# Naxaes/Rust-Swift-Raytracer

Hardware: AMD Instinct MI355X
Metric: Mrays/sec + frames/sec at 1920×1080 spp=64; 1/2/4/8 MI355X (higher is better)
Workload: dtype f32; 1 GPU; c2: 1920x1080, spp 64, depth 8, 486 spheres, 0 triangles, COUNTER RNG; width=1920, height=1080, spp=64, depth=8, parallelism=one device renders the frame in place (no RCCL call)

## Files before the change

include/raytracer_amd.h:

```cpp
#ifndef RAYTRACER_AMD_H
#define RAYTRACER_AMD_H

#include "raytracer.h"

#ifdef __cplusplus
extern "C" {
#endif

enum { RT_RNG_COUNTER = 1, RT_RNG_REPLAY = 2, RT_RNG_SERIAL = 3 };

typedef struct RtRenderOptions {
  int32_t samples_per_pixel;
  int32_t max_ray_bounces;
  uint32_t rng_mode;
  uint32_t seed;
  const uint32_t *replay_states;
  uint32_t row_block;
  uint32_t rank;
  uint32_t nranks;
  int32_t device;
  int32_t accel;
  uint32_t flags;
  int32_t ndevices;
} RtRenderOptions;
// ... 143 lines not shown
                         const void *d_records, float *d_out_rgb, void *d_out_rgba,
                         void *hip_stream);
int rt_filter_run(RtFilter *f, const RtFilterOptions *opts, const float *rgb,
                  const RtFirstHit *records, float *out_rgb, Rust_ColorU8 *out_pixels);
int rt_filter_accum(RtAccum *acc, const RtFilterOptions *opts, float *out_rgb,
                    Rust_ColorU8 *pixels);
int rt_filter_accum_device(RtAccum *acc, const RtFilterOptions *opts, float *d_out_rgb,
                           void *d_rgba, void *hip_stream);

long rt_read_samples(const Rust_WorldHandle *handle, int device, float *out, size_t n);

int rt_leaf_defer(const Rust_WorldHandle *handle, int device);

int rt_trace_plain(const Rust_WorldHandle *handle, int device);

int rt_trace_launched(const Rust_WorldHandle *handle, int device, unsigned char *out, size_t n,
                      int clear);
int rt_trace_instances(unsigned char *out, size_t n);

void rt_free_world(Rust_WorldHandle *handle);

const char *rt_last_error(void);

size_t rt_world_num_spheres(const Rust_WorldHandle *handle);
size_t rt_world_num_triangles(const Rust_WorldHandle *handle);
int rt_world_sphere(const Rust_WorldHandle *handle, size_t i, float out[10]);
int rt_world_triangle(const Rust_WorldHandle *handle, size_t i, float out[18]);
int rt_world_set_sphere_material(Rust_WorldHandle *handle, size_t i, const float material[6]);
int rt_world_set_triangle_material(Rust_WorldHandle *handle, size_t i, const float material[6]);
void rt_camera_get(const Rust_Camera *camera, float out[12]);
// ... 29 lines not shown
```

rust-swift-raytracer_amd/csrc/bvh.cpp:

```cpp
#include "bvh.h"

#include <algorithm>
#include <atomic>
#include <chrono>
#include <cmath>
#include <cstdio>
#include <cstdlib>
#include <cstring>
#include <limits>
#include <thread>

namespace rtamd {

namespace {

struct Box {
    double lo[3] = {std::numeric_limits<double>::infinity(), std::numeric_limits<double>::infinity(),
                    std::numeric_limits<double>::infinity()};
    double hi[3] = {-std::numeric_limits<double>::infinity(), -std::numeric_limits<double>::infinity(),
                    -std::numeric_limits<double>::infinity()};
    void grow(const Box &b) {
        for (int k = 0; k < 3; ++k) { lo[k] = std::min(lo[k], b.lo[k]); hi[k] = std::max(hi[k], b.hi[k]); }
    }
    void grow(const double p[3]) {
// ... 898 lines not shown
    double mag = 0;
    for (const Vec3 &v : cv) mag = std::max({mag, std::fabs((double)v.x), std::fabs((double)v.y),
                                             std::fabs((double)v.z)});
    double Mi[3][3];
    if (!(mag < 1e3) || !camera_inverse(cam, Mi)) return false;
    for (int r = 0; r < 3; ++r)
        for (int c = 0; c < 3; ++c) out.Mi[3 * r + c] = Mi[r][c];
    out.o[0] = cam.origin.x; out.o[1] = cam.origin.y; out.o[2] = cam.origin.z;
    out.e_abs = 4e-6 * (std::fabs(out.o[0]) + std::fabs(out.o[1]) + std::fabs(out.o[2]) + bv.mag);
    out.wden = (double)(float)(width - 1);
    out.hden = (double)(float)(height - 1);
    out.n = (uint32_t)n;
    out.width = (uint32_t)width;
    out.height = (uint32_t)height;
    return true;
}

PrimarySphereLists build_primary_sphere_lists(const SphereBVH &bv, const CameraModel &cam,
                                              size_t width, size_t height) {
    PrimarySphereLists out;
    const size_t n = bv.prims.size() / 4;
    if (n == 0 || n >= kSphListWalk || width < 2 || height < 2 || height > (1u << 24) ||
        width > (1u << 24) || width * height > (1ull << 28))
        return out;
    const Vec3 cv[4] = {cam.origin, cam.lower_left, cam.horizontal, cam.vertical};
    double mag = 0;
    for (const Vec3 &v : cv) mag = std::max({mag, std::fabs((double)v.x), std::fabs((double)v.y),
                                             std::fabs((double)v.z)});
    double Mi[3][3];
    if (!(mag < 1e3) || !camera_inverse(cam, Mi)) return out;
// ... 150 lines not shown
```

rust-swift-raytracer_amd/csrc/bvh.h:

```cpp
#pragma once

#include <cstdint>
#include <vector>

#include "scene.h"

namespace rtamd {

constexpr uint32_t kLeafBit = 0x80000000u;
constexpr uint32_t kNodeEnd = 0xFFFFFFFFu;

struct SphereBVH {
    std::vector<float> nodes;
    std::vector<uint32_t> miss;
    std::vector<float> prims;
    std::vector<uint32_t> prim_id;
    std::vector<uint32_t> big;
    float centre[3] = {0, 0, 0};
    float radius = 0, rmax = 0, mag = 0, inv_rmin = 0;
    uint32_t depth = 0;
    std::vector<uint32_t> corner;
};
constexpr uint32_t kCornerLeaf = 0x8000u, kCornerEnd = 0xFFFFu;
constexpr uint32_t kCornerMaxNodes = 0x7FFFu, kCornerMaxPrims = 0x1000u;
// ... 77 lines not shown
constexpr uint32_t kSphListWalk = 0xFFFFu;
struct PrimarySphereLists {
    std::vector<uint32_t> rec;
};
PrimarySphereLists build_primary_sphere_lists(const SphereBVH &bv, const CameraModel &cam,
                                              size_t width, size_t height);
struct SphereListParams {
    double Mi[9];
    double o[3];
    double e_abs, wden, hden;
    uint32_t n, width, height;
};
bool sphere_list_params(const SphereBVH &bv, const CameraModel &cam, size_t width, size_t height,
                        SphereListParams &out);

}
```

rust-swift-raytracer_amd/csrc/capi.cpp:

```cpp
#include <cstdio>
#include <cstdlib>
#include <cstring>
#include <string>

#include "../../include/raytracer.h"
#include "../../include/raytracer_amd.h"
#include "runtime.h"
#include "scene.h"

struct Rust_World {
    rtamd::WorldState state;
};
struct Rust_Camera {
    rtamd::CameraModel cam;
};
struct RtAccum {
    const Rust_WorldHandle *handle;
    rtamd::AccumState *state;
};
struct RtFilter {
    rtamd::FilterState *state;
};

namespace {
// ... 140 lines not shown
                                         static_cast<uint32_t *>(d_rgba),
                                         static_cast<hipStream_t>(hip_stream), stats);
    return rtamd::render_frame(h->world->state, h->camera->cam, width, height, o,
                               static_cast<uint32_t *>(d_rgba),
                               static_cast<hipStream_t>(hip_stream), stats);
}

int rt_trace_plain(const Rust_WorldHandle *h, int device) {
    if (!h || !h->world) {
        rtamd::set_error("rt_trace_plain: null argument");
        return -1;
    }
    return rtamd::trace_plain(h->world->state, device);
}

int rt_leaf_defer(const Rust_WorldHandle *h, int device) {
    if (!h || !h->world) {
        rtamd::set_error("rt_leaf_defer: null argument");
        return -1;
    }
    return rtamd::leaf_defer(h->world->state, device);
}

int rt_trace_launched(const Rust_WorldHandle *h, int device, unsigned char *out, size_t n, int clear) {
    if (!h || !h->world) {
        rtamd::set_error("rt_trace_launched: null argument");
        return -1;
    }
    return rtamd::trace_launched(h->world->state, device, out, n, clear != 0);
}
// ... 410 lines not shown
```

rust-swift-raytracer_amd/csrc/frame.cpp:

```cpp
#include <algorithm>
#include <cmath>
#include <cstdio>

#include "runtime_internal.h"

namespace rtamd {

size_t tile_rows(size_t height, uint32_t row_block, uint32_t rank, uint32_t nranks) {
    if (nranks <= 1) return height;
    const size_t B = row_block ? row_block : 1;
    const size_t blocks = (height + B - 1) / B;
    size_t rows = 0;
    for (size_t b = rank; b < blocks; b += nranks) rows += std::min(B, height - b * B);
    return rows;
}

size_t tile_row(size_t k, uint32_t row_block, uint32_t rank, uint32_t nranks) {
    if (nranks <= 1) return k;
    const size_t B = row_block ? row_block : 1;
    return ((k / B) * nranks + rank) * B + k % B;
}

void bind_scene_arrays(const DeviceState *d, const CameraModel &cam, size_t width, size_t height, TraceParams &p) {
    p.sph_hot = d->sph_hot.get(); p.sph_cold = d->sph_cold.get();
// ... 62 lines not shown
enum { kFrameRender = 0, kFrameNothing = 1, kFrameSerial = 2 };

struct LaunchPlan { uint64_t blocks, nwaves, chunk, parts, block_threads; };

struct FrameValues {
    uint32_t nranks = 1, B = 1;
    size_t T = 0;
    uint32_t spp = 0;
    uint64_t jobs_per_row = 0, slab_jobs = 0;
    size_t rows_per_slab = 0;
    bool fused = false, replay = false;
    bool use_bvh = false;
    const uint4 *corner_img = nullptr;
    TraceRequest want;
    bool primary_lists = false;
    bool use_tbvh = false;
    int ptl_where = 0;
    float inv_spp = 0.0f;
    bool timed = false;
    TraceVariant tv{};
    uint64_t waves_per_block = 0, full_blocks = 0, max_waves = 0;
};

struct LaunchesDone {
    LaunchPlan lean_plan{0, 0, 0, 0, 0};
    TraceVariant variant{};
    uint32_t launches = 0, waves = 0, nslab = 0;
    uint64_t samples = 0;
};

// ... 83 lines not shown
    if (f.use_bvh) {
        bind_sphere_tree(w, d, p);
        const bool lds_on = env_u64("RT_AMD_LDS", 1) != 0;
        if (lds_on && sp == nullptr && d->corner_bytes > 0 && env_u64("RT_AMD_CORNER", 1) != 0)
            f.corner_img = d->bvh_corner.get();
        f.want.corner = f.corner_img != nullptr;
        f.want.defer = f.want.corner && env_u64("RT_AMD_LEAF_DEFER", 1) != 0;
        f.want.plain = f.want.defer && d->plain_fits() && p.depth >= 1 && env_u64("RT_AMD_PLAIN", 1) != 0;
        p.use_lds = lds_on && (d->lds_bytes > 0 || f.corner_img != nullptr);
        if (d->ntri == 0 && env_u64("RT_AMD_SPHERE_LISTS", 1) != 0 && gpu_lists()) {
            bool ok = false;
            const int rc = device_sphere_lists(w, d, cam, width, height, s, ok);
            if (rc) return rc;
            p.spl = ok ? d->gspl.lists.get() : nullptr;
            f.primary_lists = ok;
        } else if (d->ntri == 0 && env_u64("RT_AMD_SPHERE_LISTS", 1) != 0 &&
                   prepare_primary_sphere_lists(w, cam, width, height)) {
            if (d->spl_version != w.spl_version) {
                HIP_TRY(replace_contents(d->spl, w.spl.rec));
                d->spl_version = w.spl_version;
            }
            p.spl = d->spl.get();
            f.primary_lists = p.spl != nullptr;
        }
    }
    return 0;
}

int bind_triangle_search(WorldState &w, DeviceState *d, const CameraModel &cam, size_t width, size_t height,
                         const RtRenderOptions &o, hipStream_t stream, hipStream_t s, FrameValues &f,
// ... 123 lines not shown
        if (const uint64_t bpc = env_u64("RT_AMD_BLOCKS_PER_CU", 0))
            if (tv.search != kSearchLdsCorner) blocks = (int)bpc;
        if (blocks < 1 && tv.lds()) { set_error("accumulation kernel does not fit its LDS tree"); return -1; }
        d->occupancy(tv) = std::max(blocks, 1);
    }
    f.waves_per_block = trace_block_threads(tv) / 64;
    f.full_blocks = (uint64_t)d->occupancy(tv) * (uint64_t)d->num_cus;
    f.max_waves = ap ? 0 : f.full_blocks * f.waves_per_block;
    p.stats = nullptr;
    if (f.timed && !ap) {
        HIP_TRY(d->stats.grow(f.max_waves * kStatSlots));
        HIP_TRY(hipMemsetAsync(d->stats.get(), 0, f.max_waves * kStatSlots * 8, s));
        p.stats = d->stats.get();
    }
    return 0;
}

hipError_t launch_recorded(DeviceState *d, TraceVariant v, const TraceParams &p, const TraceTail &tail,
                           uint32_t blocks, hipStream_t s) {
    const hipError_t e = launch_trace(v, p, tail, blocks, s);
    if (e == hipSuccess) d->trace_launched[trace_key(v)] = 1;
    return e;
}

int launch_serial_pass(DeviceState *d, size_t width, size_t height, const RtRenderOptions &o,
                       const SerialPass *sp, hipStream_t s, const FrameValues &f, TraceParams &p) {
    const uint32_t spp = f.spp;
    const uint64_t njobs = (uint64_t)sp->nsamples * sp->variants;
    if (njobs == 0) return 0;
    if (njobs > 0x7FFFFFFFull) { set_error("serial pass too large"); return -1; }
// ... 53 lines not shown

LaunchPlan plan_launch(DeviceState *d, const TraceParams &p, const FrameValues &f, TraceVariant v, uint64_t njobs) {
    const uint32_t spp = f.spp;
    const uint64_t wpb = trace_block_threads(v) / 64;
    const uint64_t jobs_per_block = wpb * 256;
    uint64_t blocks = std::min<uint64_t>((uint64_t)d->occupancy(v) * d->num_cus,
                                         (njobs + jobs_per_block - 1) / jobs_per_block);
    blocks = std::max<uint64_t>(blocks, 1);
    const uint64_t nwaves = blocks * wpb;
    uint64_t chunk = env_u64("RT_AMD_CHUNK", 0);
    if (!chunk) chunk = std::min<uint64_t>(256, std::max<uint64_t>(64, njobs / (nwaves * 16) / 64 * 64));
    chunk = chunk >= spp ? chunk / spp * spp : spp;
    if (f.fused) {
        uint64_t px = std::max<uint64_t>(1, std::min<uint64_t>(
            env_u64("RT_AMD_RESOLVE_PIX", p.step ? 1 : 8), 4096 / spp));
        while (px > 4 && njobs / (nwaves * px * spp) < 16) px /= 2;
        chunk = std::max<uint64_t>(chunk, px * spp);
    }
    uint64_t parts = env_u64("RT_AMD_PARTS", p.step ? 64 : 8);
    parts = std::max<uint64_t>(1, std::min<uint64_t>({parts, kMaxParts, njobs / (16 * chunk) + 1}));
    return LaunchPlan{blocks, nwaves, chunk, parts, wpb * 64};
}

int enqueue_launches(DeviceState *d, size_t width, size_t height, uint32_t *d_out, const AccumPass *ap,
                     hipStream_t s, const FrameValues &f, TraceParams &p, LaunchesDone &done) {
    const uint32_t spp = f.spp;
    const bool fused = f.fused, timed = f.timed, adapt = f.want.kind == kKindAdapt;
    TraceTail tail;
    tail.corner = f.corner_img;
    done.variant = f.tv;
    if (ap) {
// ... 2 lines not shown
        if (ap->n0 == 0) HIP_TRY(hipMemsetAsync(acc.sums.get(), 0, 3 * width * height * sizeof(float), s));
        tail.sums = acc.sums.get(), tail.n0 = ap->n0, tail.stride = acc.stride;
        if (adapt) tail.sumsq = acc.sumsq.get();
        if (adapt && ap->n0 == 0) {
            HIP_TRY(hipMemsetAsync(acc.sumsq.get(), 0, width * height * sizeof(float), s));
            HIP_TRY(hipMemsetAsync(acc.count.get(), 0, width * height * sizeof(uint32_t), s));
            HIP_TRY(launch_adapt_iota(const_cast<uint32_t *>(ap->list), (uint32_t)(width * height), s));
        }
    }
    const size_t units = adapt ? ap->nactive : f.T;
    const uint64_t jobs_per_unit = adapt ? spp : f.jobs_per_row;
    done.samples = (uint64_t)units * jobs_per_unit;
    const size_t units_per_slab =
        adapt ? (size_t)std::min<uint64_t>(std::max<uint64_t>(1, f.slab_jobs / spp), std::max<size_t>(units, 1))
              : f.rows_per_slab;
    uint32_t &nslab = done.nslab;
    for (size_t r0 = 0; r0 < units; r0 += units_per_slab, ++nslab) {
        const size_t rows = std::min(units_per_slab, units - r0);
        hipEvent_t *ev3 = nullptr;
        if (timed) {
            while (d->tev.size() < 3 * (size_t)(nslab + 1)) {
                hipEvent_t e;
                HIP_TRY(hipEventCreate(&e));
                d->tev.push_back(e);
            }
            ev3 = &d->tev[3 * (size_t)nslab];
        }
        const uint64_t njobs = rows * jobs_per_unit;
        p.slab_row0 = adapt ? 0u : (uint32_t)r0;
        p.gj32 = f.nranks == 1 && (uint64_t)width * height * spp < (1ull << 32) ? 1u : 0u;
        p.gj_c0 = (uint32_t)(((uint64_t)height - 1 - r0) * width * spp);
        p.gj_2p = (uint32_t)(2ull * width * spp);
        if (ap) p.gj32 = (uint64_t)width * height * ap->acc->stride < (1ull << 32) ? 1u : 0u;
// ... 124 lines not shown
    bind_scene(d, cam, width, height, o, sp, d_replay, f, p);
    rc = bind_sphere_search(w, d, cam, width, height, o, sp, s, f, p);
    if (rc) return rc;
    rc = bind_triangle_search(w, d, cam, width, height, o, stream, s, f, p);
    if (rc) return rc;
    const uint32_t nheld = ap ? ap->n0 + f.spp : f.spp;
    f.inv_spp = ap ? 1.0f / (float)nheld
                   : 1.0f / (float)o.samples_per_pixel;
    p.inv_spp = f.inv_spp;
    p.alpha_u8 = alpha_byte(nheld, f.inv_spp);
    p.out = d_out;
    f.timed = stats != nullptr;
    rc = choose_kernel_instance(d, sp, ap, s, f, p);
    if (rc) return rc;
    if (sp) return launch_serial_pass(d, width, height, o, sp, s, f, p);

    LaunchesDone done;
    rc = enqueue_launches(d, width, height, d_out, ap, s, f, p, done);
    if (rc) return rc;
    if (!f.timed) return 0;
    rc = queue_frame_stats(d, s, f, p, done);
    if (rc || defer_stats) return rc;
    return collect_frame_stats(d, stats);
}

int collect_frame_stats(DeviceState *d, RtRenderStats *stats) {
    auto &pd = d->pend;
    if (!pd.active) {
        set_error("no counted frame pending on this device");
        return -1;
    }
    pd.active = false;
    HIP_TRY(hipSetDevice(d->device));
    HIP_TRY(hipStreamSynchronize(pd.stream));
// ... 74 lines not shown
    std::lock_guard<std::recursive_mutex> lock(w.mu);
    DeviceState *d = nullptr;
    int rc = device_for(w, device, d);
    if (rc) return rc;
    return d->last_leaf_defer;
}

int trace_plain(WorldState &w, int device) {
    std::lock_guard<std::recursive_mutex> lock(w.mu);
    DeviceState *d = nullptr;
    int rc = device_for(w, device, d);
    if (rc) return rc;
    return d->last_plain ? 1 : 0;
}

int trace_launched(WorldState &w, int device, uint8_t *out, size_t n, bool clear) {
    std::lock_guard<std::recursive_mutex> lock(w.mu);
    DeviceState *d = nullptr;
    int rc = device_for(w, device, d);
    if (rc) return rc;
    if (out) std::memcpy(out, d->trace_launched, std::min<size_t>(n, kTraceKeys));
    if (clear) std::memset(d->trace_launched, 0, sizeof(d->trace_launched));
    return kTraceKeys;
}

int trace_instances(uint8_t *out, size_t n) {
    for (int key = 0; key < kTraceKeys && (size_t)key < n && out; ++key)
        out[key] = trace_instance_exists(key) ? 1 : 0;
    return kTraceKeys;
}
// ... 81 lines not shown
```

rust-swift-raytracer_amd/csrc/primary_lists.cpp:

```cpp
#include <chrono>

#include "runtime_internal.h"

namespace rtamd {

static uint32_t cam_leaf() {
    return (uint32_t)env_u64("RT_AMD_CAM_LEAF", 2);
}

void prepare_camera(WorldState &w, const CameraModel &cam, bool tree) {
    if (w.tbvh.nodes.empty() || env_u64("RT_AMD_CAMERA_TREE", 1) == 0) return;
    const float o[3] = {cam.origin.x, cam.origin.y, cam.origin.z};
    if (w.ctree_version && std::memcmp(o, w.ctree.origin, sizeof(o)) == 0 && (w.ctree_full || !tree)) return;
    w.ctree = build_camera_triangle_bvh(w.scene.triangles, w.packed.tri_hot, w.tbvh, o, cam_leaf(), tree);
    w.ctree_full = tree;
    ++w.ctree_version;
}

static bool sync_lists() { return env_u64("RT_AMD_SYNC_LISTS", 0) != 0; }
bool gpu_lists() { return env_u64("RT_AMD_GPU_LISTS", 1) != 0; }

template <typename T>
static bool job_ready(const std::future<T> &f) {
    return f.valid() && f.wait_for(std::chrono::seconds(0)) == std::future_status::ready;
// ... 58 lines not shown
                std::vector<uint32_t> dev(2 * width * height);
                HIP_TRY(hipMemcpyAsync(dev.data(), g.lists.get(), dev.size() * 4, hipMemcpyDeviceToHost, s));
                HIP_TRY(hipStreamSynchronize(s));
                for (size_t px = 0; px < width * height; ++px) {
                    const bool same = h.rec.empty()
                                          ? (dev[2 * px + 1] >> 16) == kSphListWalk
                                          : dev[2 * px] == h.rec[2 * px] && dev[2 * px + 1] == h.rec[2 * px + 1];
                    if (!same) {
                        set_error("RT_AMD_SPL_CHECK: device sphere lists differ from the host build at pixel " +
                                  std::to_string(px));
                        return -2;
                    }
                }
            }
        }
        g.remember(cam, width, height);
    }
    ok = g.ok;
    return 0;
}

bool gpu_tri_lists() { return env_u64("RT_AMD_GPU_TRI_LISTS", 1) != 0; }

int device_tri_lists(WorldState &w, DeviceState *d, const CameraModel &cam, size_t width, size_t height,
                     hipStream_t s, bool &ok) {
    auto &g = d->gptl;
    if (!g.current(cam, width, height, w.ctree_version)) {
        const CameraTriangleBVH &ct = w.ctree;
        TriListParams tp;
        g.built = false;
        g.ok = tri_list_params(ct, cam, width, height, tp);
        g.host = g.ok && ((height + 15) / 16 > 65535 ||
                                      (uint64_t)tp.strips_per_row * height >= 0x7FFFFFFFull);
        if (g.host) g.ok = false;
// ... 62 lines not shown
```

rust-swift-raytracer_amd/csrc/render.h:

```cpp
#pragma once

#include <hip/hip_runtime.h>

#include <cstdint>

#include "fastdiv.h"

namespace rtamd {

enum : uint32_t { kRngCounter = 1, kRngReplay = 2 };
enum : uint32_t { kRngSerialCount = 3, kRngSerialEstimate = 4, kRngSerialCheck = 5, kRngSerialCoalesce = 6,
                  kRngSerialPixel = 7 };
enum : uint32_t { kMatDiffuse = 0, kMatMetal = 1, kMatDielectric = 2, kMatEmission = 3 };
constexpr uint32_t kPrimaryTriStripW = 8;
#ifndef RT_TRACE_RING
#define RT_TRACE_RING 4
#endif
constexpr uint32_t kTraceRing = RT_TRACE_RING;
#ifdef RT_STAMPS
constexpr uint32_t kStatSlots = 24;
#else
constexpr uint32_t kStatSlots = 16;
#endif
constexpr uint32_t kStampSegs = 8;
// ... 170 lines not shown
    float *sums = nullptr, *sumsq = nullptr;
    const uint32_t *list = nullptr;
    uint32_t n0 = 0, stride = 0;
};
hipError_t launch_trace(TraceVariant v, const TraceParams &p, const TraceTail &tail, uint32_t blocks,
                        hipStream_t stream);
int trace_leaf_defer(TraceVariant v);
enum : uint32_t { kViewNormal = 0, kViewDepth = 1, kViewAlbedo = 2, kViewPrim = 3, kViewNone = 0xFFFFFFFFu };
struct FirstHitTail {
    void *out;
    float su, sv;
    uint32_t x0, y0, w, h;
    uint32_t view;
};
hipError_t launch_first_hit(const TraceParams &p, const FirstHitTail &tail, hipStream_t stream);
struct FilterPack {
    const float *rgb;
    const float *sums;
    size_t plane;
    const uint32_t *count;
    uint32_t held;
    const float4 *records;
    float sigma_z;
    float4 *col, *g0, *g1;
    uint32_t npix;
};
hipError_t launch_filter_pack(const FilterPack &a, hipStream_t stream);
struct FilterLevel {
    const float4 *cin, *g0, *g1;
    float4 *cout;
// ... 89 lines not shown
```

rust-swift-raytracer_amd/csrc/runtime.h:

```cpp
#pragma once

#include <hip/hip_runtime.h>

#include <cstdint>
#include <cstring>
#include <future>
#include <map>
#include <mutex>
#include <memory>
#include <string>
#include <vector>

#include "bvh.h"
#include "device_buffer.h"
#include "render.h"
#include "scene.h"

struct RtRenderOptions;
struct RtRenderStats;
struct RtFirstHitOptions;
struct RtFilterOptions;

namespace rtamd {

// ... 32 lines not shown
    DevBuf<uint4> cam_nodes;
    DevBuf<float4> cam_tris;
    uint32_t cam_nnodes = 0;
    uint64_t cam_version = 0;
    DevBuf<uint32_t> ptl_off, ptl_items;
    uint64_t ptl_version = 0;
    DevBuf<uint2> spl;
    uint64_t spl_version = 0;
    struct DeviceSphereLists {
        DevBuf<uint2> lists;
        DevBuf<int4> rects;
        DevBuf<uint32_t> flag;
        CameraModel cam{};
        size_t w = 0, h = 0;
        bool built = false, ok = false;
        bool current(const CameraModel &c, size_t width, size_t height) const {
            return built && w == width && h == height && std::memcmp(&cam, &c, sizeof(c)) == 0;
        }
        void remember(const CameraModel &c, size_t width, size_t height) {
            cam = c;
            w = width;
            h = height;
            built = true;
        }
    } gspl;
    struct DeviceTriLists {
        DevBuf<float> box;
        uint64_t box_version = 0;
        DevBuf<uint32_t> off, items;
        DevBuf<int4> rects;
// ... 63 lines not shown
    struct PendingStats {
        bool active = false;
        size_t nrec = 0;
        uint32_t nslab = 0;
        uint32_t launches = 0;
        uint64_t samples = 0;
        bool use_bvh = false, use_tbvh = false;
        RtRenderStatsFixed fixed;
        hipStream_t stream = nullptr;
    } pend;
    size_t last_jobs = 0;
    size_t last_spp = 0;
    bool last_fused = false;
    int last_leaf_defer = 0;
    bool last_plain = false;
    uint8_t trace_launched[kTraceKeys] = {};
    ~DeviceState();
};

struct AccumState;

struct WorldState {
    SceneModel scene;
    PackedScene packed;
    SphereBVH bvh;
    TriangleBVH tbvh;
    TriangleCells tcells;
    CameraTriangleBVH ctree;
    uint64_t ctree_version = 0;
    bool ctree_full = false;
// ... 128 lines not shown
                       RtRenderStats *stats);

int assemble_tiles(const uint32_t *gathered, uint32_t *out, size_t width, size_t height, uint32_t row_block,
                   uint32_t nranks, size_t max_rows, hipStream_t stream);

int comm_count(int first, int n);

int render_frame_host(WorldState &w, const CameraModel &cam, size_t width, size_t height,
                      const RtRenderOptions &opts, void *host_out, RtRenderStats *stats);

void prepare_camera(WorldState &w, const CameraModel &cam, bool tree = false);

long read_samples(WorldState &w, int device, float *out, size_t n);
int leaf_defer(WorldState &w, int device);
int trace_plain(WorldState &w, int device);
int trace_launched(WorldState &w, int device, uint8_t *out, size_t n, bool clear);
int trace_instances(uint8_t *out, size_t n);
int primary_tri_lists(WorldState &w, int device);

size_t tile_rows(size_t height, uint32_t row_block, uint32_t rank, uint32_t nranks);
size_t tile_row(size_t k, uint32_t row_block, uint32_t rank, uint32_t nranks);

}
```

rust-swift-raytracer_amd/csrc/runtime_internal.h:

```cpp
#pragma once

#include <cstdlib>
#include <cstring>
#include <string>
#include <vector>

#include <rccl/rccl.h>

#include "../../include/raytracer_amd.h"
#include "runtime.h"

namespace rtamd {

#define HIP_TRY(expr)                                                                 \
    do {                                                                              \
        hipError_t e_ = (expr);                                                       \
        if (e_ != hipSuccess) {                                                       \
            set_error(std::string(#expr) + " failed: " + hipGetErrorString(e_));      \
            return -2;                                                                \
        }                                                                             \
    } while (0)

#define NCCL_TRY(expr)                                                                \
    do {                                                                              \
// ... 20 lines not shown

int device_for(WorldState &w, int want, DeviceState *&out);

void bind_scene_arrays(const DeviceState *d, const CameraModel &cam, size_t width, size_t height, TraceParams &p);
void bind_sphere_tree(const WorldState &w, const DeviceState *d, TraceParams &p);
void bind_triangle_tree(const WorldState &w, const DeviceState *d, TraceParams &p);
int bind_primary_triangle_search(WorldState &w, DeviceState *d, const CameraModel &cam, size_t width, size_t height,
                                 int32_t accel, hipStream_t stream, hipStream_t s, TraceParams &p);

bool gpu_lists();
bool gpu_tri_lists();
void prepare_camera_lists(WorldState &w, const CameraModel &cam, size_t width, size_t height, bool lists);
bool prepare_primary_sphere_lists(WorldState &w, const CameraModel &cam, size_t width, size_t height);
int device_sphere_lists(WorldState &w, DeviceState *d, const CameraModel &cam, size_t width, size_t height,
                        hipStream_t s, bool &ok);
int device_tri_lists(WorldState &w, DeviceState *d, const CameraModel &cam, size_t width, size_t height,
                     hipStream_t s, bool &ok);

int serial_check_args(size_t width, size_t height, const RtRenderOptions &o);
int serial_find_states(WorldState &w, const CameraModel &cam, size_t width, size_t height,
                       const RtRenderOptions &o, DeviceState *d, hipStream_t s, RtRenderStats *stats);

WorldState *accum_begin(AccumState &a, const CameraModel &cam, std::unique_lock<std::recursive_mutex> &lock);

int device_list(int first, int n, std::vector<int> &devs);

}
```

rust-swift-raytracer_amd/raytracer_amd.py:

```python
from __future__ import annotations

import ctypes as C
import os
import subprocess

import numpy as np

HERE = os.path.dirname(os.path.abspath(__file__))
LIB_PATH = os.environ.get("RT_AMD_LIB") or os.path.join(HERE, "lib", "libraytracer.so")

RNG_COUNTER, RNG_REPLAY, RNG_SERIAL = 1, 2, 3
ACCEL_AUTO, ACCEL_BRUTE, ACCEL_BVH = 0, 1, 2
FLAG_KEEP_SAMPLES = 1
FLAG_SERIAL_CHECK = 2
DEFAULT_SEED = 2547549
VIEW_NORMAL, VIEW_DEPTH, VIEW_ALBEDO, VIEW_PRIM = 0, 1, 2, 3
FILTER_SAME_PRIM = 1

EXPORTS = (
    "load_world", "render", "move_camera_position",
    "rt_default_options", "rt_tile_rows", "rt_tile_row", "rt_sample_seed", "rt_render_ex",
    "rt_render_device", "rt_read_samples", "rt_free_world", "rt_last_error", "rt_world_num_spheres",
    "rt_world_num_triangles", "rt_world_sphere", "rt_world_triangle", "rt_camera_get",
    "rt_last_parse_error", "rt_write_ppm", "rt_device_count", "rt_comm_count",
    "rt_world_set_sphere_material", "rt_world_set_triangle_material", "rt_assemble_tiles",
    "rt_accum_default_options", "rt_accum_create", "rt_accum_add", "rt_accum_add_device",
    "rt_accum_samples", "rt_accum_read", "rt_accum_reset", "rt_accum_free",
    "rt_adapt_default_options", "rt_adapt_enable", "rt_adapt_disable", "rt_adapt_active",
    "rt_adapt_read_counts", "rt_adapt_read_sumsq", "rt_adapt_read_active", "rt_leaf_defer",
    "rt_trace_plain", "rt_trace_launched", "rt_trace_instances",
    "rt_camera_new_with_vertical_fov", "rt_camera_new_look_at", "rt_camera_from_floats",
    "rt_camera_translate", "rt_camera_free", "rt_primary_tri_lists", "rt_camera_record_builds",
    "rt_first_hit_default_options", "rt_first_hit", "rt_first_hit_device", "rt_first_hit_pick",
    "rt_first_hit_view", "rt_first_hit_view_device",
    "rt_filter_default_options", "rt_filter_create", "rt_filter_free", "rt_filter_run_device",
    "rt_filter_run", "rt_filter_accum", "rt_filter_accum_device",
)


class RenderError(RuntimeError):
    pass


class ColorU8(C.Structure):
    _fields_ = [("r", C.c_uint8), ("g", C.c_uint8), ("b", C.c_uint8), ("a", C.c_uint8)]
# ... 127 lines not shown
        L.rt_last_parse_error.restype = C.c_int
        L.rt_write_ppm.restype = C.c_int
        L.rt_write_ppm.argtypes = [C.POINTER(CFramebuffer), C.c_char_p]
        L.rt_device_count.restype = C.c_int
        L.rt_comm_count.restype = C.c_int
        L.rt_comm_count.argtypes = [C.c_int, C.c_int]
        L.rt_assemble_tiles.restype = C.c_int
        L.rt_assemble_tiles.argtypes = [C.c_void_p, C.c_void_p, C.c_size_t, C.c_size_t, C.c_uint32,
                                        C.c_uint32, C.c_size_t, C.c_void_p]
        if hasattr(L, "rt_leaf_defer"):
            L.rt_leaf_defer.restype = C.c_int
            L.rt_leaf_defer.argtypes = [H, C.c_int]
        if hasattr(L, "rt_trace_plain"):
            L.rt_trace_plain.restype = C.c_int
            L.rt_trace_plain.argtypes = [H, C.c_int]
        if hasattr(L, "rt_trace_launched"):
            L.rt_trace_launched.restype = C.c_int
            L.rt_trace_launched.argtypes = [H, C.c_int, C.POINTER(C.c_uint8), C.c_size_t, C.c_int]
            L.rt_trace_instances.restype = C.c_int
            L.rt_trace_instances.argtypes = [C.POINTER(C.c_uint8), C.c_size_t]
        if hasattr(L, "rt_camera_new_look_at"):
            L.rt_camera_new_with_vertical_fov.restype = C.c_void_p
            L.rt_camera_new_with_vertical_fov.argtypes = [fp, C.c_float, C.c_float]
            L.rt_camera_new_look_at.restype = C.c_void_p
            L.rt_camera_new_look_at.argtypes = [fp, fp, fp, C.c_float, C.c_float]
            L.rt_camera_from_floats.restype = C.c_void_p
            L.rt_camera_from_floats.argtypes = [fp]
            L.rt_camera_translate.restype = C.c_void_p
            L.rt_camera_translate.argtypes = [C.c_void_p, C.c_float, C.c_float, C.c_float]
            L.rt_camera_free.restype = None
# ... 264 lines not shown
            raise RenderError(f"rt_read_samples failed ({n}): {self._L.rt_last_error().decode()}")
        return out[: n // 4]

    def leaf_defer(self, device=-1):
        n = self._L.rt_leaf_defer(self._h, device)
        if n < 0:
            raise RenderError(f"rt_leaf_defer failed ({n}): {self._L.rt_last_error().decode()}")
        return n

    def trace_plain(self, device=-1):
        n = self._L.rt_trace_plain(self._h, device)
        if n < 0:
            raise RenderError(f"rt_trace_plain failed ({n}): {self._L.rt_last_error().decode()}")
        return n

    def trace_launched(self, clear=False, device=-1):
        out = np.zeros(self._L.rt_trace_instances(None, 0), np.uint8)
        n = self._L.rt_trace_launched(self._h, device, out.ctypes.data_as(C.POINTER(C.c_uint8)), out.size,
                                      1 if clear else 0)
        if n < 0:
            raise RenderError(f"rt_trace_launched failed ({n}): {self._L.rt_last_error().decode()}")
        return out

    def render_device(self, width, height, out_ptr: int, stream_ptr: int = 0, spp=16, depth=8,
                      mode=RNG_COUNTER, seed=DEFAULT_SEED, row_block=8, rank=0, nranks=1,
                      device=-1, accel=ACCEL_AUTO, stats=True, keep_samples=False, ndevices=0,
                      serial_check=False):
        o, _ = options(spp, depth, mode, seed, None, row_block, rank, nranks, device, accel,
                       keep_samples, self._L, ndevices, serial_check)
        st = RenderStats()
# ... 233 lines not shown
```

Measured before the change: 73390 Mrays/s.

## Classify sky-only rows on host and shade them with a cheap sky kernel

Adds a conservative host classification that projects every sphere's bounding box into screen space and tests big spheres analytically to find top and bottom image rows whose primary rays can only hit the sky. Those rows are rendered by a new lightweight kernel that only evaluates the sky gradient per sample, and the main trace launches skip them. The goal is to avoid full BVH traversal for pixels that cannot hit geometry. Classification runs lazily after the first frame's launches and is reused while the camera is unchanged, so the saving starts from the next frame. The error margins in the classification are what keep the result bit-identical. A knob for the minimum chunks per wave is also exposed.

```diff
diff --git a/include/raytracer_amd.h b/include/raytracer_amd.h
--- a/include/raytracer_amd.h
+++ b/include/raytracer_amd.h
@@ -181,6 +181,8 @@
 
 int rt_trace_plain(const Rust_WorldHandle *handle, int device);
 
+int rt_sky_rows(const Rust_WorldHandle *handle, int device);
+
 int rt_trace_launched(const Rust_WorldHandle *handle, int device, unsigned char *out, size_t n,
                       int clear);
 int rt_trace_instances(unsigned char *out, size_t n);
diff --git a/rust-swift-raytracer_amd/csrc/bvh.cpp b/rust-swift-raytracer_amd/csrc/bvh.cpp
--- a/rust-swift-raytracer_amd/csrc/bvh.cpp
+++ b/rust-swift-raytracer_amd/csrc/bvh.cpp
@@ -7,6 +7,7 @@
 #include <cstdio>
 #include <cstdlib>
 #include <cstring>
+#include <functional>
 #include <limits>
 #include <thread>
 
@@ -936,6 +937,166 @@
     out.width = (uint32_t)width;
     out.height = (uint32_t)height;
     return true;
+}
+
+namespace {
+
+int sphere_list_rect(const SphereBVH &bv, uint32_t i, const SphereListParams &sp, int64_t rect[4]) {
+    const float *s = &bv.prims[(size_t)i * 4];
+    const double *o = sp.o;
+    const double c[3] = {s[0], s[1], s[2]};
+    const double r = std::sqrt((double)s[3]) * (1 + 1e-6);
+    const double a = std::sqrt((c[0] - o[0]) * (c[0] - o[0]) + (c[1] - o[1]) * (c[1] - o[1]) +
+                               (c[2] - o[2]) * (c[2] - o[2]));
+    const double R = r + 2 * 3e-3 * (a + r) * 1.01 + 2 * sp.e_abs;
+    if (!std::isfinite(R) || !std::isfinite(a)) return -1;
+    double umin = 1e300, umax = -1e300, vmin = 1e300, vmax = -1e300;
+    int front = 0, behind = 0;
+    for (int k = 0; k < 8; ++k) {
+        const double P[3] = {c[0] + (k & 1 ? R : -R) - o[0], c[1] + (k & 2 ? R : -R) - o[1],
+                             c[2] + (k & 4 ? R : -R) - o[2]};
+        double w[3];
+        for (int q = 0; q < 3; ++q) w[q] = sp.Mi[3 * q] * P[0] + sp.Mi[3 * q + 1] * P[1] + sp.Mi[3 * q + 2] * P[2];
+        const double wn = std::fabs(w[0]) + std::fabs(w[1]) + std::fabs(w[2]);
+        if (w[2] > 1e-6 * wn) {
+            ++front;
+            umin = std::min(umin, w[0] / w[2]); umax = std::max(umax, w[0] / w[2]);
+            vmin = std::min(vmin, w[1] / w[2]); vmax = std::max(vmax, w[1] / w[2]);
+        } else if (w[2] < -1e-6 * wn) {
+            ++behind;
+        }
+    }
+    if (behind == 8) return 0;
+    if (front < 8) return -1;
+    const int64_t W = sp.width, H = sp.height;
+    const double cl = std::floor(umin * sp.wden) - 2, ch = std::floor(umax * sp.wden) + 1;
+    const double rl = std::floor(vmin * sp.hden) - 2, rh = std::floor(vmax * sp.hden) + 1;
+    if (ch < 0 || cl > (double)(W - 1) || rh < 0 || rl > (double)(H - 1)) return 0;
+    rect[0] = std::max<int64_t>(0, (int64_t)cl); rect[1] = std::min<int64_t>(W - 1, (int64_t)ch);
+    rect[2] = std::max<int64_t>(0, (int64_t)rl); rect[3] = std::min<int64_t>(H - 1, (int64_t)rh);
+    return 1;
+}
+
+bool big_sphere_clear(const double oc[3], double kappa, double away, const double L[3], const double h[3],
+                      const double vv[3], double u0, double u1, double v0, double v1) {
+    const double *c[3] = {h, vv, L};
+    double ac[3], Q[3][3], G[3][3];
+    for (int i = 0; i < 3; ++i) ac[i] = oc[0] * c[i][0] + oc[1] * c[i][1] + oc[2] * c[i][2];
+    for (int i = 0; i < 3; ++i)
+        for (int j = 0; j < 3; ++j) {
+            G[i][j] = c[i][0] * c[j][0] + c[i][1] * c[j][1] + c[i][2] * c[j][2];
+            Q[i][j] = ac[i] * ac[j] - kappa * G[i][j];
+        }
+    struct P2 { double u, v; };
+    const P2 rect[4] = {{u0, v0}, {u1, v0}, {u1, v1}, {u0, v1}};
+    double max_len = 0;
+    for (const P2 &p : rect)
+        max_len = std::max(max_len, std::sqrt(G[0][0] * p.u * p.u + G[1][1] * p.v * p.v + G[2][2] +
+                                              2 * (G[0][1] * p.u * p.v + G[0][2] * p.u + G[1][2] * p.v)));
+    const double lim = away * max_len;
+    auto toward = [&](const P2 &p) { return lim - (ac[0] * p.u + ac[1] * p.v + ac[2]); };
+    P2 poly[8];
+    int n = 0;
+    for (int k = 0; k < 4; ++k) {
+        const P2 &p = rect[k], &q = rect[(k + 1) & 3];
+        const double tp = toward(p), tq = toward(q);
+        if (tp >= 0) poly[n++] = p;
+        if ((tp >= 0) != (tq >= 0)) {
+            const double t = tp / (tp - tq);
+            poly[n++] = P2{p.u + t * (q.u - p.u), p.v + t * (q.v - p.v)};
+        }
+    }
+    if (n == 0) return !std::isnan(lim + toward(rect[0]));
+    auto g = [&](const P2 &p) {
+        return Q[0][0] * p.u * p.u + Q[1][1] * p.v * p.v + Q[2][2] +
+               2 * (Q[0][1] * p.u * p.v + Q[0][2] * p.u + Q[1][2] * p.v);
+    };
+    double m = -1e300;
+    for (int k = 0; k < n; ++k) {
+        const P2 &p = poly[k], &q = poly[(k + 1) % n];
+        const P2 mid{0.5 * (p.u + q.u), 0.5 * (p.v + q.v)};
+        const double g0 = g(p), gh = g(mid), g1 = g(q);
+        m = std::max({m, g0, gh, g1});
+        if (std::isnan(g0 + gh + g1)) return false;
+        const double A = 2 * (g1 + g0 - 2 * gh), B = g1 - g0 - A;
+        if (A < 0) {
+            const double t = -B / (2 * A);
+            if (t > 0 && t < 1) m = std::max(m, g(P2{p.u + t * (q.u - p.u), p.v + t * (q.v - p.v)}));
+        }
+    }
+    const double det = Q[0][0] * Q[1][1] - Q[0][1] * Q[0][1];
+    if (det != 0) {
+        const P2 s{(Q[0][1] * Q[1][2] - Q[1][1] * Q[0][2]) / det, (Q[0][1] * Q[0][2] - Q[0][0] * Q[1][2]) / det};
+        if (s.u > u0 && s.u < u1 && s.v > v0 && s.v < v1 && toward(s) >= 0) m = std::max(m, g(s));
+    }
+    return m < 0;
+}
+
+}
+
+SkyRows classify_sky_rows(const SphereBVH &bv, const std::vector<Sphere> &spheres, const CameraModel &cam,
+                          size_t width, size_t height) {
+    SphereListParams sp;
+    if (!sphere_list_params(bv, cam, width, height, sp)) return SkyRows{};
+    for (const Sphere &s : spheres)
+        if (!finite_sphere(s) || !std::isfinite(s.radius * s.radius)) return SkyRows{};
+    const int64_t W = (int64_t)width, H = (int64_t)height;
+    std::vector<uint8_t> covered(height, 0);
+    for (uint32_t i = 0; i < sp.n; ++i) {
+        int64_t rect[4];
+        const int rc = sphere_list_rect(bv, i, sp, rect);
+        if (rc < 0) return SkyRows{};
+        if (rc > 0) std::fill(covered.begin() + rect[2], covered.begin() + rect[3] + 1, (uint8_t)1);
+    }
+    int64_t top = 0, bottom = 0;
+    while (top < H && !covered[H - 1 - top]) ++top;
+    while (top + bottom < H && !covered[bottom]) ++bottom;
+    if (!bv.big.empty() && top + bottom > 0) {
+        const Vec3 cv[4] = {cam.origin, cam.lower_left, cam.horizontal, cam.vertical};
+        double S = 0;
+        for (const Vec3 &v : cv) S += std::fabs((double)v.x) + std::fabs((double)v.y) + std::fabs((double)v.z);
+        const double e_dir = 0x1p-20 * S;
+        double eps[3];
+        for (int q = 0; q < 3; ++q)
+            eps[q] = e_dir * (std::fabs(sp.Mi[3 * q]) + std::fabs(sp.Mi[3 * q + 1]) + std::fabs(sp.Mi[3 * q + 2]));
+        if (!(eps[2] < 0.25)) return SkyRows{};
+        const double du = (eps[0] + 2 * eps[2]) / (1 - eps[2]), dv = (eps[1] + 2 * eps[2]) / (1 - eps[2]);
+        if (!(du <= 0.5 / sp.wden) || !(dv <= 0.5 / sp.hden)) return SkyRows{};
+        const double o[3] = {cam.origin.x, cam.origin.y, cam.origin.z};
+        const double L[3] = {cam.lower_left.x - o[0], cam.lower_left.y - o[1], cam.lower_left.z - o[2]};
+        const double h[3] = {cam.horizontal.x, cam.horizontal.y, cam.horizontal.z};
+        const double vv[3] = {cam.vertical.x, cam.vertical.y, cam.vertical.z};
+        const double u0 = -1.0 / sp.wden, u1 = (double)(W + 1) / sp.wden;
+        for (uint32_t id : bv.big) {
+            const Sphere &s = spheres[id];
+            const double oc[3] = {o[0] - s.center.x, o[1] - s.center.y, o[2] - s.center.z};
+            const double N = oc[0] * oc[0] + oc[1] * oc[1] + oc[2] * oc[2];
+            const double E = 0x1p-18 * N;
+            const double kappa = N - (double)s.radius * (double)s.radius - E;
+            if (!(kappa > 0) || !(N < 1e30)) return SkyRows{};
+            const double away = 0x1p-20 * std::sqrt(N);
+            auto clear = [&](int64_t lo, int64_t hi) {
+                return big_sphere_clear(oc, kappa, away, L, h, vv, u0, u1, (double)(lo - 1) / sp.hden,
+                                        (double)(hi + 1) / sp.hden);
+            };
+            std::function<int64_t(int64_t, int64_t, bool)> run = [&](int64_t lo, int64_t hi, bool from_top) -> int64_t {
+                if (lo >= hi) return 0;
+                if (clear(lo, hi)) return hi - lo;
+                if (hi - lo == 1) return 0;
+                const int64_t mid = (lo + hi) / 2;
+                const int64_t a0 = from_top ? mid : lo, a1 = from_top ? hi : mid;
+                const int64_t n = run(a0, a1, from_top);
+                if (n < a1 - a0) return n;
+                return n + (from_top ? run(lo, mid, true) : run(mid, hi, false));
+            };
+            top = run(H - top, H, true);
+            bottom = run(0, std::min(bottom, H - top), false);
+        }
+    }
+    SkyRows out;
+    out.top = (uint32_t)top;
+    out.bottom = (uint32_t)std::min(bottom, H - top);
+    return out;
 }
 
 PrimarySphereLists build_primary_sphere_lists(const SphereBVH &bv, const CameraModel &cam,
diff --git a/rust-swift-raytracer_amd/csrc/bvh.h b/rust-swift-raytracer_amd/csrc/bvh.h
--- a/rust-swift-raytracer_amd/csrc/bvh.h
+++ b/rust-swift-raytracer_amd/csrc/bvh.h
@@ -115,4 +115,8 @@
 bool sphere_list_params(const SphereBVH &bv, const CameraModel &cam, size_t width, size_t height,
                         SphereListParams &out);
 
+struct SkyRows { uint32_t top = 0, bottom = 0; };
+SkyRows classify_sky_rows(const SphereBVH &bv, const std::vector<Sphere> &spheres, const CameraModel &cam,
+                          size_t width, size_t height);
+
 }
diff --git a/rust-swift-raytracer_amd/csrc/capi.cpp b/rust-swift-raytracer_amd/csrc/capi.cpp
--- a/rust-swift-raytracer_amd/csrc/capi.cpp
+++ b/rust-swift-raytracer_amd/csrc/capi.cpp
@@ -178,6 +178,14 @@
     return rtamd::trace_plain(h->world->state, device);
 }
 
+int rt_sky_rows(const Rust_WorldHandle *h, int device) {
+    if (!h || !h->world) {
+        rtamd::set_error("rt_sky_rows: null argument");
+        return -1;
+    }
+    return rtamd::sky_rows(h->world->state, device);
+}
+
 int rt_leaf_defer(const Rust_WorldHandle *h, int device) {
     if (!h || !h->world) {
         rtamd::set_error("rt_leaf_defer: null argument");
diff --git a/rust-swift-raytracer_amd/csrc/frame.cpp b/rust-swift-raytracer_amd/csrc/frame.cpp
--- a/rust-swift-raytracer_amd/csrc/frame.cpp
+++ b/rust-swift-raytracer_amd/csrc/frame.cpp
@@ -100,6 +100,8 @@
     const uint4 *corner_img = nullptr;
     TraceRequest want;
     bool primary_lists = false;
+    SkyRows dev_sky;
+    SkyRows sky;
     bool use_tbvh = false;
     int ptl_where = 0;
     float inv_spp = 0.0f;
@@ -213,6 +215,7 @@
             if (rc) return rc;
             p.spl = ok ? d->gspl.lists.get() : nullptr;
             f.primary_lists = ok;
+            if (ok) f.dev_sky = d->gspl.sky;
         } else if (d->ntri == 0 && env_u64("RT_AMD_SPHERE_LISTS", 1) != 0 &&
                    prepare_primary_sphere_lists(w, cam, width, height)) {
             if (d->spl_version != w.spl_version) {
@@ -366,6 +369,15 @@
         p.stats = d->stats.get();
     }
     return 0;
+}
+
+void choose_sky_rows(const DeviceState *d, const SerialPass *sp, const AccumPass *ap, FrameValues &f,
+                     const TraceParams &p) {
+    f.sky = SkyRows{};
+    if (sp || ap || f.timed || !f.fused || f.replay || f.nranks != 1 || d->ntri != 0 || !f.use_bvh ||
+        !f.primary_lists || p.depth < 1 || p.ablate != 0 || env_u64("RT_AMD_SKY_ROWS", 1) == 0)
+        return;
+    f.sky = f.dev_sky;
 }
 
 hipError_t launch_recorded(DeviceState *d, TraceVariant v, const TraceParams &p, const TraceTail &tail,
@@ -449,7 +461,8 @@
     if (f.fused) {
         uint64_t px = std::max<uint64_t>(1, std::min<uint64_t>(
             env_u64("RT_AMD_RESOLVE_PIX", p.step ? 1 : 8), 4096 / spp));
-        while (px > 4 && njobs / (nwaves * px * spp) < 16) px /= 2;
+        const uint64_t min_chunks = env_u64("RT_AMD_CHUNKS_PER_WAVE", 16);
+        while (px > 4 && njobs / (nwaves * px * spp) < min_chunks) px /= 2;
         chunk = std::max<uint64_t>(chunk, px * spp);
     }
     uint64_t parts = env_u64("RT_AMD_PARTS", p.step ? 64 : 8);
@@ -482,9 +495,12 @@
     const size_t units_per_slab =
         adapt ? (size_t)std::min<uint64_t>(std::max<uint64_t>(1, f.slab_jobs / spp), std::max<size_t>(units, 1))
               : f.rows_per_slab;
+    const size_t row_lo = f.sky.top, row_hi = units - f.sky.bottom;
+    d->last_sky_rows = f.sky.top + f.sky.bottom;
+    if (d->last_sky_rows) HIP_TRY(launch_sky_rows(p, f.sky.top, f.sky.bottom, s));
     uint32_t &nslab = done.nslab;
-    for (size_t r0 = 0; r0 < units; r0 += units_per_slab, ++nslab) {
-        const size_t rows = std::min(units_per_slab, units - r0);
+    for (size_t r0 = row_lo; r0 < row_hi; r0 += units_per_slab, ++nslab) {
+        const size_t rows = std::min(units_per_slab, row_hi - r0);
         hipEvent_t *ev3 = nullptr;
         if (timed) {
             while (d->tev.size() < 3 * (size_t)(nslab + 1)) {
@@ -639,10 +655,12 @@
     rc = choose_kernel_instance(d, sp, ap, s, f, p);
     if (rc) return rc;
     if (sp) return launch_serial_pass(d, width, height, o, sp, s, f, p);
+    choose_sky_rows(d, sp, ap, f, p);
 
     LaunchesDone done;
     rc = enqueue_launches(d, width, height, d_out, ap, s, f, p, done);
     if (rc) return rc;
+    classify_pending_sky_rows(w, d);
     if (!f.timed) return 0;
     rc = queue_frame_stats(d, s, f, p, done);
     if (rc || defer_stats) return rc;
@@ -747,6 +765,14 @@
     return d->last_plain ? 1 : 0;
 }
 
+int sky_rows(WorldState &w, int device) {
+    std::lock_guard<std::recursive_mutex> lock(w.mu);
+    DeviceState *d = nullptr;
+    int rc = device_for(w, device, d);
+    if (rc) return rc;
+    return (int)d->last_sky_rows;
+}
+
 int trace_launched(WorldState &w, int device, uint8_t *out, size_t n, bool clear) {
     std::lock_guard<std::recursive_mutex> lock(w.mu);
     DeviceState *d = nullptr;
diff --git a/rust-swift-raytracer_amd/csrc/primary_lists.cpp b/rust-swift-raytracer_amd/csrc/primary_lists.cpp
--- a/rust-swift-raytracer_amd/csrc/primary_lists.cpp
+++ b/rust-swift-raytracer_amd/csrc/primary_lists.cpp
@@ -96,10 +96,19 @@
                 }
             }
         }
+        g.sky = SkyRows{};
+        g.sky_pending = g.ok;
         g.remember(cam, width, height);
     }
     ok = g.ok;
     return 0;
+}
+
+void classify_pending_sky_rows(WorldState &w, DeviceState *d) {
+    auto &g = d->gspl;
+    if (!g.sky_pending) return;
+    g.sky = classify_sky_rows(w.bvh, w.scene.spheres, g.cam, g.w, g.h);
+    g.sky_pending = false;
 }
 
 bool gpu_tri_lists() { return env_u64("RT_AMD_GPU_TRI_LISTS", 1) != 0; }
diff --git a/rust-swift-raytracer_amd/csrc/render.h b/rust-swift-raytracer_amd/csrc/render.h
--- a/rust-swift-raytracer_amd/csrc/render.h
+++ b/rust-swift-raytracer_amd/csrc/render.h
@@ -208,6 +208,7 @@
     uint32_t view;
 };
 hipError_t launch_first_hit(const TraceParams &p, const FirstHitTail &tail, hipStream_t stream);
+hipError_t launch_sky_rows(const TraceParams &p, uint32_t top, uint32_t bottom, hipStream_t stream);
 struct FilterPack {
     const float *rgb;
     const float *sums;
diff --git a/rust-swift-raytracer_amd/csrc/runtime.h b/rust-swift-raytracer_amd/csrc/runtime.h
--- a/rust-swift-raytracer_amd/csrc/runtime.h
+++ b/rust-swift-raytracer_amd/csrc/runtime.h
@@ -70,6 +70,8 @@
         CameraModel cam{};
         size_t w = 0, h = 0;
         bool built = false, ok = false;
+        SkyRows sky;
+        bool sky_pending = false;
         bool current(const CameraModel &c, size_t width, size_t height) const {
             return built && w == width && h == height && std::memcmp(&cam, &c, sizeof(c)) == 0;
         }
@@ -163,6 +165,7 @@
     bool last_fused = false;
     int last_leaf_defer = 0;
     bool last_plain = false;
+    uint32_t last_sky_rows = 0;
     uint8_t trace_launched[kTraceKeys] = {};
     ~DeviceState();
 };
@@ -321,6 +324,7 @@
 long read_samples(WorldState &w, int device, float *out, size_t n);
 int leaf_defer(WorldState &w, int device);
 int trace_plain(WorldState &w, int device);
+int sky_rows(WorldState &w, int device);
 int trace_launched(WorldState &w, int device, uint8_t *out, size_t n, bool clear);
 int trace_instances(uint8_t *out, size_t n);
 int primary_tri_lists(WorldState &w, int device);
diff --git a/rust-swift-raytracer_amd/csrc/runtime_internal.h b/rust-swift-raytracer_amd/csrc/runtime_internal.h
--- a/rust-swift-raytracer_amd/csrc/runtime_internal.h
+++ b/rust-swift-raytracer_amd/csrc/runtime_internal.h
@@ -58,6 +58,7 @@
 bool prepare_primary_sphere_lists(WorldState &w, const CameraModel &cam, size_t width, size_t height);
 int device_sphere_lists(WorldState &w, DeviceState *d, const CameraModel &cam, size_t width, size_t height,
                         hipStream_t s, bool &ok);
+void classify_pending_sky_rows(WorldState &w, DeviceState *d);
 int device_tri_lists(WorldState &w, DeviceState *d, const CameraModel &cam, size_t width, size_t height,
                      hipStream_t s, bool &ok);
 
diff --git a/rust-swift-raytracer_amd/csrc/sky.hip b/rust-swift-raytracer_amd/csrc/sky.hip
--- /dev/null
+++ b/rust-swift-raytracer_amd/csrc/sky.hip
@@ -0,0 +1,73 @@
+#include <hip/hip_runtime.h>
+
+#include <cstdint>
+
+#include "exactdiv.h"
+#include "kernels.h"
+#include "render.h"
+
+#pragma clang fp contract(off)
+
+#include "chunk_resolve.h"
+#include "device_math.h"
+
+namespace rtamd {
+namespace {
+
+struct SkyParams {
+    TraceParams p;
+    uint32_t top, bottom;
+};
+
+constexpr uint32_t kSkyThreads = 256;
+
+__global__ __launch_bounds__(kSkyThreads) void sky_rows_kernel(SkyParams a) {
+    const TraceParams &p = a.p;
+    const uint32_t i = blockIdx.x * kSkyThreads + threadIdx.x;
+    if (i >= (a.top + a.bottom) * p.width) return;
+    const uint32_t q = fdiv(i, p.div_width);
+    const uint32_t col = i - q * p.width;
+    const uint32_t trow = q < a.top ? q : p.height - a.bottom + (q - a.top);
+    const uint32_t row = p.height - 1u - trow;
+    const uint64_t gjob0 = ((uint64_t)row * p.width + col) * p.spp;
+    const F3 h = f3(p.cam[6], p.cam[7], p.cam[8]);
+    const F3 vv = f3(p.cam[9], p.cam[10], p.cam[11]);
+    const F3 org = f3(p.cam[0], p.cam[1], p.cam[2]);
+    const F3 llc = f3(p.cam[3], p.cam[4], p.cam[5]);
+    const bool xd = p.xdiv_uv != 0;
+    float acc_r = 0.0f, acc_g = 0.0f, acc_b = 0.0f;
+    for (uint32_t s = 0; s < p.spp; ++s) {
+        uint32_t rng = counter_seed(p.seed, gjob0 + s);
+        const float un = draw_plus(rng, (float)col);
+        const float vn = draw_plus(rng, (float)row);
+        const float u = xd ? xdiv(un, p.wden, p.wrcp) : un / p.wden;
+        const float v = xd ? xdiv(vn, p.hden, p.hrcp) : vn / p.hden;
+        const F3 vdir = ((llc + scale(h, u)) + scale(vv, v)) - org;
+        const F3 dir = unit<true>(vdir);
+        const F3 un3 = unit<true>(dir);
+        const float t = 0.5f * (un3.y + 1.0f);
+        const float w = 1.0f - t;
+        acc_r = acc_r + (1.0f * w + 0.5f * t);
+        acc_g = acc_g + (1.0f * w + 0.7f * t);
+        acc_b = acc_b + (1.0f * w + 1.0f * t);
+    }
+    p.out[(size_t)trow * p.width + col] = resolve_channel(p, acc_r) | (resolve_channel(p, acc_g) << 8) |
+                                          (resolve_channel(p, acc_b) << 16) | (p.alpha_u8 << 24);
+}
+
+}
+
+hipError_t launch_sky_rows(const TraceParams &p, uint32_t top, uint32_t bottom, hipStream_t stream) {
+    if (p.out == nullptr || p.width == 0 || (uint64_t)top + bottom > p.height || p.mode != kRngCounter ||
+        p.depth < 1 || p.nranks != 1)
+        return hipErrorInvalidValue;
+    const uint64_t npix = ((uint64_t)top + bottom) * p.width;
+    if (npix == 0) return hipSuccess;
+    const uint64_t blocks = (npix + kSkyThreads - 1) / kSkyThreads;
+    if (npix > 0xFFFFFFFFull || blocks > 0x7FFFFFFFull) return hipErrorInvalidValue;
+    SkyParams a{p, top, bottom};
+    void *args[] = {(void *)&a};
+    return hipLaunchKernel((const void *)sky_rows_kernel, dim3((uint32_t)blocks), dim3(kSkyThreads), args, 0, stream);
+}
+
+}
diff --git a/rust-swift-raytracer_amd/raytracer_amd.py b/rust-swift-raytracer_amd/raytracer_amd.py
--- a/rust-swift-raytracer_amd/raytracer_amd.py
+++ b/rust-swift-raytracer_amd/raytracer_amd.py
@@ -28,7 +28,7 @@
     "rt_accum_samples", "rt_accum_read", "rt_accum_reset", "rt_accum_free",
     "rt_adapt_default_options", "rt_adapt_enable", "rt_adapt_disable", "rt_adapt_active",
     "rt_adapt_read_counts", "rt_adapt_read_sumsq", "rt_adapt_read_active", "rt_leaf_defer",
-    "rt_trace_plain", "rt_trace_launched", "rt_trace_instances",
+    "rt_trace_plain", "rt_trace_launched", "rt_trace_instances", "rt_sky_rows",
     "rt_camera_new_with_vertical_fov", "rt_camera_new_look_at", "rt_camera_from_floats",
     "rt_camera_translate", "rt_camera_free", "rt_primary_tri_lists", "rt_camera_record_builds",
     "rt_first_hit_default_options", "rt_first_hit", "rt_first_hit_device", "rt_first_hit_pick",
@@ -186,6 +186,9 @@
         if hasattr(L, "rt_trace_plain"):
             L.rt_trace_plain.restype = C.c_int
             L.rt_trace_plain.argtypes = [H, C.c_int]
+        if hasattr(L, "rt_sky_rows"):
+            L.rt_sky_rows.restype = C.c_int
+            L.rt_sky_rows.argtypes = [H, C.c_int]
         if hasattr(L, "rt_trace_launched"):
             L.rt_trace_launched.restype = C.c_int
             L.rt_trace_launched.argtypes = [H, C.c_int, C.POINTER(C.c_uint8), C.c_size_t, C.c_int]
@@ -480,6 +483,12 @@
             raise RenderError(f"rt_trace_plain failed ({n}): {self._L.rt_last_error().decode()}")
         return n
 
+    def sky_rows(self, device=-1):
+        n = self._L.rt_sky_rows(self._h, device)
+        if n < 0:
+            raise RenderError(f"rt_sky_rows failed ({n}): {self._L.rt_last_error().decode()}")
+        return n
+
     def trace_launched(self, clear=False, device=-1):
         out = np.zeros(self._L.rt_trace_instances(None, 0), np.uint8)
         n = self._L.rt_trace_launched(self._h, device, out.ctypes.data_as(C.POINTER(C.c_uint8)), out.size,
```

Result: faster. 76570 Mrays/s (median of 6 runs) (+4.3%).
